# uber-research/deep-neuroevolution

Hardware: NVIDIA H100
Metric: env-steps/sec across ES population (whole box) (higher is better)
Workload: dtype f32

## Files before the change

### deep-neuroevolution_b200/csrc/conv_s2d.cu

```cuda
#include "common.cuh"
#include "forward.cuh"
#include "epilogue.cuh"
#include "wgmma.cuh"

using namespace wg;

namespace {

constexpr int S2D_MMA_THREADS = 256;
constexpr int S2D_CONV_WARPS = 4;
constexpr int S2D_CONV_THREADS = S2D_CONV_WARPS * 32;
constexpr int S2D_THREADS = 512;
constexpr int S2D_REGS_MMA = 176, S2D_REGS_AUX = 80;
constexpr int S2D_FRAME_BYTES = 84 * 84 * 4;
constexpr int S2D_FRAME_STRIDE = (S2D_FRAME_BYTES + 127) / 128 * 128;
constexpr int S2D_MAX_GROUPS = 8;
constexpr int S2D_MAX_BST = 8;
constexpr int S2D_SMEM_BUDGET = 222 * 1024;

constexpr int cmin(int a, int b) { return a < b ? a : b; }
constexpr int cmax(int a, int b) { return a > b ? a : b; }

struct S2dGeom {
    int S, PADB, W, KT, CIN, CP, NG, NPIX, PIXP, PARTS, LBO, GROUP_BYTES, IMG_BYTES, HIN;
};
__host__ __device__ constexpr S2dGeom s2d_geom(int CIN, int KS, int S, int HIN, int HOUT, int PAD, bool in_u8) {
    S2dGeom g{};
    const int HP = (HOUT - 1) * S + KS;
    g.S = S; g.PADB = PAD; g.W = HP / S; g.KT = KS / S; g.CIN = CIN; g.CP = S * S * CIN; g.NG = g.CP / 16;
    g.NPIX = g.W * g.W; g.PIXP = (g.NPIX + 7) / 8 * 8; g.PARTS = in_u8 ? 1 : 2; g.LBO = g.PIXP * 16;
    g.GROUP_BYTES = g.PARTS * 2 * g.LBO; g.IMG_BYTES = g.NG * g.GROUP_BYTES; g.HIN = HIN;
    return g;
}

constexpr int s2d_taps_per_chunk(int ntap, int piece_stride) {
    int best = 1;
    for (int t = 1; t <= ntap; ++t)
        if (ntap % t == 0 && 2 * t * piece_stride <= 26000) best = t;
    return best;
}

template <int CIN, int COUT, int KS, int S, int HIN, int HOUT, int PAD, bool IN_U8>
struct S2dCfg {
    static constexpr S2dGeom G = s2d_geom(CIN, KS, S, HIN, HOUT, PAD, IN_U8);
    static_assert(((HOUT - 1) * S + KS) % S == 0 && KS % S == 0, "space-to-depth needs S | KS and S | padded size");
    static_assert(CIN % 4 == 0 && COUT % 16 == 0 && G.CP % 16 == 0 && G.NG <= S2D_MAX_GROUPS, "tile constraints");
    static constexpr int W = G.W, KT = G.KT, NTAP = KT * KT, NG = G.NG, PIXP = G.PIXP, LBO_A = G.LBO;
    static constexpr int PARTS = G.PARTS, GROUP_BYTES = G.GROUP_BYTES, IMG_BYTES = G.IMG_BYTES;
    static constexpr int MMAX = (HOUT - 1) * (W + 1);
    static constexpr int MT = MMAX / 64 + 1;
    static constexpr int NTW = (MT + 1) / 2;
    static constexpr int ACC = COUT / 2;
    static_assert(2 * NTW * ACC <= 128, "accumulators exceed the MMA warpgroups' register budget");
    static constexpr int MAXOFF = (KT - 1) * (W + 1);
    static constexpr int REACH = MT * 64 + MAXOFF;
    static constexpr int SLACK = REACH > PIXP ? ((REACH - PIXP) * 16 + 127) / 128 * 128 : 0;
    static constexpr int A_REGION = IMG_BYTES + SLACK;
    static constexpr int LBO_B = 2 * COUT * 16;
    static constexpr int PIECE = 16 * COUT * 4;
    static constexpr int PIECE_STRIDE = PIECE + 16;
    static constexpr int TPC = s2d_taps_per_chunk(NTAP, PIECE_STRIDE);
    static constexpr int NCPG = NTAP / TPC;
    static constexpr int NCH = NG * NCPG;
    static constexpr int B_TILE = TPC * 2 * LBO_B;
    static constexpr int RAW_BYTES = 2 * TPC * PIECE_STRIDE;
    static constexpr int BST_BYTES = (cmax(B_TILE, RAW_BYTES) + 127) / 128 * 128;
    static constexpr int FRAME_REGION = IN_U8 ? 2 * S2D_FRAME_STRIDE : 0;
    static constexpr int NSTB = cmin(S2D_MAX_BST, (S2D_SMEM_BUDGET - A_REGION - FRAME_REGION - 256) / BST_BYTES);
    static_assert(NSTB >= 2, "shared memory: B ring too shallow");
    static constexpr int SMEM_BYTES = A_REGION + NSTB * BST_BYTES + FRAME_REGION + 256;
    static constexpr int B_UNITS = COUT * TPC * 2;
    static constexpr int NGRP = 2;
    static constexpr int WPG = S2D_CONV_WARPS / NGRP, TG = 32 * WPG;
    static constexpr int B_UPT = (B_UNITS + TG - 1) / TG;
    static_assert(TG % COUT == 0 && NCH % NGRP == 0, "B unit map: a thread keeps its column; groups alternate chunks");
    static_assert(!IN_U8 || NCPG == 1, "the uint8 frame is staged per channel group by the group's (only) chunk");
};

struct S2dOut {
    float* base;
    int64_t slot_stride;
    int next_img;
    int nS, nPADB, nW, nPIXP, nHP;
    float* xc;
    int xc_ko;
};

__device__ __forceinline__ void store_split_pair(uint4* p_hi, uint4* p_lo, int word, float v0, float v1) {
    uint32_t hi, lo;
    split_f16x2(v0, v1, hi, lo);
    reinterpret_cast<uint32_t*>(p_hi)[word] = hi;
    reinterpret_cast<uint32_t*>(p_lo)[word] = lo;
}

template <int COUT, int HOUT, int W, int MT, int NTW, int ACC, bool IN_U8, int MODE, bool FAST>
__device__ __forceinline__ void s2d_epilogue(const float (&acc)[NTW][ACC], const float (&cor)[NTW][ACC], int w, int wq, int lane,
                                             const float* sb, const float* sm, const float* si, const float* sg, const float* se,
                                             int act, bool bn, const S2dOut& so, float* outp, int slot) {
    constexpr float IN_SCALE = IN_U8 ? (1.0f / 255.0f) : 1.0f;
    const bool next_img = MODE < 0 ? so.next_img != 0 : MODE > 0;
    const int nS = MODE > 0 ? MODE : so.nS;
#pragma unroll
    for (int j = 0; j < NTW; ++j) {
        const int t = w + 2 * j;
        if (t >= MT) continue;
#pragma unroll
        for (int h = 0; h < 2; ++h) {
            const int m = t * 64 + wq * 16 + (lane >> 2) + 8 * h;
            const int oy = m / W, ox = m - oy * W;
            if (oy >= HOUT || ox >= HOUT) continue;
#pragma unroll
            for (int i = 0; i < COUT / 8; ++i) {
                const int n = 8 * i + 2 * (lane & 3);
                float v[2];
#pragma unroll
                for (int e = 0; e < 2; ++e) {
                    float r = fmaf(cor[j][4 * i + 2 * h + e], F16_LO_INV, acc[j][4 * i + 2 * h + e]);
                    if (IN_U8) r *= IN_SCALE;
                    r += sb[n + e];
                    if (FAST) {
                        v[e] = fmaxf(r, 0.0f);
                    } else {
                        if (bn) r = (r - sm[n + e]) * si[n + e] * sg[n + e] + se[n + e];
                        v[e] = act == DNE_ACT_RELU ? fmaxf(r, 0.0f) : (act == DNE_ACT_TANH ? tanhf(r) : r);
                    }
                }
                if (!next_img) {
                    *reinterpret_cast<float2*>(outp + (int64_t)(oy * HOUT + ox) * COUT + n) = make_float2(v[0], v[1]);
                    if (so.xc) {
                        const int ko = ((oy * HOUT + ox) * COUT + 8 * i) >> 3;
                        uint4* xp = reinterpret_cast<uint4*>(so.xc) + ((int64_t)(slot >> 7) * so.xc_ko + ko) * 256 + (slot & 127);
                        store_split_pair(xp, xp + 128, lane & 3, v[0], v[1]);
                    }
                } else {
                    const int Y = oy + so.nPADB, X = ox + so.nPADB;
                    const int pix = (Y / nS) * so.nW + (X / nS);
                    const int pp = (Y % nS) * nS + (X % nS);
                    const int co = pp * (COUT / 8) + i;
                    uint4* p = reinterpret_cast<uint4*>(outp) + (size_t)((co >> 1) * 4 + (co & 1)) * so.nPIXP + pix;
                    store_split_pair(p, p + (size_t)2 * so.nPIXP, lane & 3, v[0], v[1]);
                }
            }
        }
    }
}

template <int CIN, int COUT, int KS, int S, int HIN, int HOUT, int PAD, bool IN_U8>
__global__ void __launch_bounds__(S2D_THREADS, 1)
conv_s2d_kernel(SlotArgs sa, int64_t off_w, LayerEpi epi, const void* __restrict__ in_base, int64_t in_slot_stride,
                S2dOut so, int n_slots, int vdiv, int in_mod) {
    using Cfg = S2dCfg<CIN, COUT, KS, S, HIN, HOUT, PAD, IN_U8>;
    constexpr int NG = Cfg::NG, NSTB = Cfg::NSTB, MT = Cfg::MT, NTW = Cfg::NTW, W = Cfg::W, KT = Cfg::KT;
    constexpr int TPC = Cfg::TPC, NCPG = Cfg::NCPG, NCH = Cfg::NCH;
    extern __shared__ uint8_t smem_raw[];
    uint8_t* smem = (uint8_t*)(((uintptr_t)smem_raw + 127) & ~(uintptr_t)127);
    __shared__ uint64_t a_full[NG], a_empty[NG], raw_full[NSTB], b_full[NSTB], b_empty[NSTB];
    __shared__ uint64_t frame_full[2], frame_empty[2];
    __shared__ __align__(16) float s_bias[2][COUT], s_mean[2][COUT], s_inv[2][COUT], s_gamma[2][COUT], s_beta[2][COUT];

    const int tid = threadIdx.x, warp = tid >> 5, lane = tid & 31;
    pdl_trigger();
    const uint32_t sA = smem_u32(smem), sB = sA + Cfg::A_REGION;
    uint8_t* const gB = smem + Cfg::A_REGION;
    uint8_t* const gFrame = gB + NSTB * Cfg::BST_BYTES;

    if (tid == 0) {
        for (int i = 0; i < NG; ++i) {
            mbar_init(&a_full[i], IN_U8 ? Cfg::WPG : 1);
            mbar_init(&a_empty[i], S2D_MMA_THREADS);
        }
        for (int i = 0; i < NSTB; ++i) {
            mbar_init(&raw_full[i], 1);
            mbar_init(&b_full[i], Cfg::WPG);
            mbar_init(&b_empty[i], S2D_MMA_THREADS);
        }
        for (int i = 0; i < 2; ++i) {
            mbar_init(&frame_full[i], 1);
            mbar_init(&frame_empty[i], S2D_CONV_WARPS);
        }
        fence_mbar_init();
    }
    __syncthreads();
    if (warp < 8) regs_inc<S2D_REGS_MMA>();
    else regs_dec<S2D_REGS_AUX>();

    if (warp < 8) {
        const int w = warp >> 2, wq = warp & 3;
        const int et = tid;
        const int act = epi.act;
        const bool bn = epi.bn != DNE_BN_NONE;
        float acc[NTW][Cfg::ACC], cor[NTW][Cfg::ACC];
        uint32_t cb = 0, it = 0;
        pdl_wait();
        for (int slot = blockIdx.x; slot < n_slots; slot += gridDim.x) {
            const int ms = slot / vdiv;
            if (!slot_active(sa, ms)) continue;
            const uint32_t pb = it & 1;
            {
                const float* th = slot_theta(sa, ms);
                const int64_t idx = sa.noise_idx[ms];
                const float s = sa.scale[ms];
                for (int c = et; c < COUT; c += S2D_MMA_THREADS) {
                    const ChanEpi ce = make_chan_epi(sa, epi, ms, COUT, c, th, idx, s);
                    s_bias[pb][c] = ce.bias; s_mean[pb][c] = ce.mean; s_inv[pb][c] = ce.inv; s_gamma[pb][c] = ce.gamma; s_beta[pb][c] = ce.beta;
                }
            }
            float* outp = so.base + slot * so.slot_stride;
            if (so.next_img) {
                const int nHP = so.nHP, no = COUT / 8;
                for (int b = et; b < nHP * nHP; b += S2D_MMA_THREADS) {
                    const int Y = b / nHP, X = b - Y * nHP;
                    if (Y >= so.nPADB && Y < so.nPADB + HOUT && X >= so.nPADB && X < so.nPADB + HOUT) continue;
                    const int pix = (Y / so.nS) * so.nW + (X / so.nS), pp = (Y % so.nS) * so.nS + (X % so.nS);
                    for (int q = 0; q < no; ++q) {
                        const int co = pp * no + q;
                        uint4* p = reinterpret_cast<uint4*>(outp) + (size_t)((co >> 1) * 4 + (co & 1)) * so.nPIXP + pix;
                        p[0] = make_uint4(0u, 0u, 0u, 0u);
                        p[(size_t)2 * so.nPIXP] = make_uint4(0u, 0u, 0u, 0u);
                    }
                }
            }
            for (int c = 0; c < NCH; ++c, ++cb) {
                const int g = c / NCPG, tc = c - g * NCPG;
                const uint32_t st = cb % NSTB;
                if (tc == 0) mbar_wait(&a_full[g], it & 1);
                mbar_wait(&b_full[st], (cb / NSTB) & 1);
                wgmma_fence();
#pragma unroll
                for (int tl = 0; tl < TPC; ++tl) {
                    const int tap = tc * TPC + tl;
                    const int toff = (tap / KT) * W + (tap % KT);
                    const uint64_t dB = smem_desc(sB + st * Cfg::BST_BYTES + tl * 2 * Cfg::LBO_B, Cfg::LBO_B, 128);
#pragma unroll
                    for (int j = 0; j < NTW; ++j) {
                        const int t = min(w + 2 * j, MT - 1);
                        const uint64_t dA = smem_desc(sA + g * Cfg::GROUP_BYTES + (t * 64 + toff) * 16, Cfg::LBO_A, 128);
                        const uint32_t first = (c | tl) != 0;
                        wgmma_f16<COUT>(acc[j], dA, dB, first);
                        wgmma_f16<COUT>(cor[j], dA, dB + (uint64_t)((COUT * 16) >> 4), first);
                        if (!IN_U8) wgmma_f16<COUT>(cor[j], dA + (uint64_t)((2 * Cfg::LBO_A) >> 4), dB, 1);
                    }
                }
                wgmma_commit();
                wgmma_wait<1>();
                if (c > 0) {
                    const int pg = (c - 1) / NCPG;
                    mbar_arrive(&b_empty[(cb - 1) % NSTB]);
                    if ((c - 1) - pg * NCPG == NCPG - 1) mbar_arrive(&a_empty[pg]);
                }
            }
            wgmma_wait<0>();
#pragma unroll
            for (int j = 0; j < NTW; ++j) {
                fence_regs<Cfg::ACC>(acc[j]);
                fence_regs<Cfg::ACC>(cor[j]);
            }
            mbar_arrive(&b_empty[(cb - 1) % NSTB]);
            mbar_arrive(&a_empty[NG - 1]);
            named_bar_sync(2, S2D_MMA_THREADS);
            {
                const float *sb = s_bias[pb], *sm = s_mean[pb], *si = s_inv[pb], *sg = s_gamma[pb], *se = s_beta[pb];
                const bool relu_only = !bn && act == DNE_ACT_RELU;
#define S2D_EPI(MODE, FAST)                                                                                              \
    s2d_epilogue<COUT, HOUT, W, MT, NTW, Cfg::ACC, IN_U8, MODE, FAST>(acc, cor, w, wq, lane, sb, sm, si, sg, se, act, bn, so, \
                                                                       outp, slot)
                constexpr int FAST_MODE = CIN == 32 ? 1 : 0;
                if (!IN_U8 && relu_only && (FAST_MODE == 0 ? !so.next_img : (so.next_img && so.nS == FAST_MODE)))
                    S2D_EPI(FAST_MODE, true);
                else S2D_EPI(-1, false);
#undef S2D_EPI
            }
            ++it;
        }
    } else if (warp == 12) {
        if (lane == 0) {
            pdl_wait();
            uint32_t it = 0;
            for (int slot = blockIdx.x; slot < n_slots; slot += gridDim.x) {
                if (!slot_active(sa, slot / vdiv)) continue;
                if (IN_U8) {
                    const uint32_t fb = it & 1;
                    mbar_wait(&frame_empty[fb], ((it >> 1) & 1) ^ 1);
                    mbar_arrive_expect_tx(&frame_full[fb], S2D_FRAME_BYTES);
                    const int fslot = in_mod > 0 ? slot % in_mod : slot;
                    bulk_g2s(gFrame + fb * S2D_FRAME_STRIDE, (const uint8_t*)in_base + fslot * in_slot_stride, S2D_FRAME_BYTES,
                             &frame_full[fb]);
                } else {
                    const uint8_t* src = (const uint8_t*)((const float*)in_base + slot * in_slot_stride);
                    for (int g = 0; g < NG; ++g) {
                        mbar_wait(&a_empty[g], (it & 1) ^ 1);
                        mbar_arrive_expect_tx(&a_full[g], Cfg::GROUP_BYTES);
                        bulk_g2s(smem + g * Cfg::GROUP_BYTES, src + (size_t)g * Cfg::GROUP_BYTES, Cfg::GROUP_BYTES, &a_full[g]);
                    }
                }
                ++it;
            }
        }
    } else if (warp == 13) {
        if (lane == 0) {
            uint32_t cb = 0;
            for (int slot = blockIdx.x; slot < n_slots; slot += gridDim.x) {
                const int ms = slot / vdiv;
                if (!slot_active(sa, ms)) continue;
                const float* th = slot_theta(sa, ms) + off_w;
                const float* nz = sa.noise + sa.noise_idx[ms] + off_w;
                const int a_t = (int)(((uintptr_t)th >> 2) & 3), a_n = (int)(((uintptr_t)nz >> 2) & 3);
                for (int c = 0; c < NCH; ++c, ++cb) {
                    const int g = c / NCPG, tc = c - g * NCPG;
                    const uint32_t st = cb % NSTB;
                    mbar_wait(&b_empty[st], ((cb / NSTB) & 1) ^ 1);
                    mbar_arrive_expect_tx(&raw_full[st], Cfg::RAW_BYTES);
                    uint8_t* dst = gB + st * Cfg::BST_BYTES;
                    const int cp = 16 * g, pp = cp / CIN, ci = cp % CIN, py = pp / S, px = pp % S;
#pragma unroll
                    for (int tl = 0; tl < TPC; ++tl) {
                        const int tap = tc * TPC + tl;
                        const int ty = tap / KT, tx = tap % KT;
                        const int kk = ((ty * S + py) * KS + (tx * S + px)) * CIN + ci;
                        bulk_g2s(dst + tl * Cfg::PIECE_STRIDE, th + (int64_t)kk * COUT - a_t, Cfg::PIECE_STRIDE, &raw_full[st]);
                        bulk_g2s(dst + (TPC + tl) * Cfg::PIECE_STRIDE, nz + (int64_t)kk * COUT - a_n, Cfg::PIECE_STRIDE, &raw_full[st]);
                    }
                }
            }
        }
    } else if (warp < 12) {
        constexpr int TG = Cfg::TG, NGRP = Cfg::NGRP;
        const int ct = tid - S2D_MMA_THREADS;
        const int grp = ct / TG, tg = ct - grp * TG;
        {
            constexpr int Z0 = IN_U8 ? 0 : Cfg::IMG_BYTES, Z1 = Cfg::A_REGION;
            for (int i = Z0 / 16 + ct; i < Z1 / 16; i += S2D_CONV_THREADS) sts128(sA + i * 16, make_float4(0.f, 0.f, 0.f, 0.f));
            fence_proxy_async_smem();
            named_bar_sync(1, S2D_CONV_THREADS);
        }
        const int n = tg % COUT;
        constexpr int KQ_STEP = TG / COUT;
        const int kq0 = tg / COUT;
        uint32_t it = 0;
        for (int slot = blockIdx.x; slot < n_slots; slot += gridDim.x) {
            const int ms = slot / vdiv;
            if (!slot_active(sa, ms)) continue;
            const float* th = slot_theta(sa, ms) + off_w;
            const float* nz = sa.noise + sa.noise_idx[ms] + off_w;
            const int a_t = (int)(((uintptr_t)th >> 2) & 3), a_n = (int)(((uintptr_t)nz >> 2) & 3);
            const float s = sa.scale[ms];
            if (IN_U8) mbar_wait(&frame_full[it & 1], (it >> 1) & 1);
            for (int c = grp; c < NCH; c += NGRP) {
                const int g = c / NCPG;
                const uint32_t cb = it * NCH + c, st = cb % NSTB;
                if (IN_U8) {
                    static_assert(!IN_U8 || (CIN == 4 && S == 4 && HIN == 84), "uint8 staging is written for the 84x84x4 frame stack, stride 4");
                    const uint32_t frame = smem_u32(gFrame + (it & 1) * S2D_FRAME_STRIDE);
                    const int py = g;
                    mbar_wait(&a_empty[g], (it & 1) ^ 1);
                    for (int u = tg; u < 2 * W * W; u += TG) {
                        const int h = u / (W * W), pix = u - h * (W * W);
                        const int yq = pix / W, xq = pix - yq * W;
                        const int y = 4 * yq + py - PAD, x0 = 4 * xq + 2 * h - PAD;
                        if (y >= 0 && y < HIN && x0 >= 0 && x0 < HIN) {
                            uint32_t p0, p1;
                            asm volatile("ld.shared.v2.u32 {%0, %1}, [%2];" : "=r"(p0), "=r"(p1) : "r"(frame + (y * HIN + x0) * 4));
                            auto h2 = [](uint32_t lo8, uint32_t hi8) {
                                return (uint32_t)__half_as_ushort(__ushort2half_rn((unsigned short)lo8)) |
                                       ((uint32_t)__half_as_ushort(__ushort2half_rn((unsigned short)hi8)) << 16);
                            };
                            const uint4 row = make_uint4(h2(p0 & 255u, (p0 >> 8) & 255u), h2((p0 >> 16) & 255u, p0 >> 24),
                                                         h2(p1 & 255u, (p1 >> 8) & 255u), h2((p1 >> 16) & 255u, p1 >> 24));
                            sts128u(sA + g * Cfg::GROUP_BYTES + h * Cfg::LBO_A + pix * 16, row);
                        }
                    }
                    fence_proxy_async_smem();
                    __syncwarp();
                    if (lane == 0) {
                        mbar_arrive(&a_full[g]);
                        if (c + NGRP >= NCH) mbar_arrive(&frame_empty[it & 1]);
                    }
                }
                mbar_wait(&raw_full[st], (cb / NSTB) & 1);
                const uint32_t sBs = sB + st * Cfg::BST_BYTES;
                float w[Cfg::B_UPT][8];
#pragma unroll
                for (int i = 0; i < Cfg::B_UPT; ++i) {
                    const int kp = kq0 + i * KQ_STEP;
                    if (kp < TPC * 2) {
                        const uint32_t pt = sBs + (kp >> 1) * Cfg::PIECE_STRIDE + (uint32_t)((a_t + (8 * (kp & 1)) * COUT + n) * 4);
                        const uint32_t pn = sBs + (TPC + (kp >> 1)) * Cfg::PIECE_STRIDE + (uint32_t)((a_n + (8 * (kp & 1)) * COUT + n) * 4);
#pragma unroll
                        for (int j = 0; j < 8; ++j) w[i][j] = perturbed(lds32(pt + j * COUT * 4), s, lds32(pn + j * COUT * 4));
                    }
                }
                named_bar_sync(3 + grp, TG);
#pragma unroll
                for (int i = 0; i < Cfg::B_UPT; ++i) {
                    const int kp = kq0 + i * KQ_STEP;
                    if (kp < TPC * 2) {
                        uint4 hi, lo;
                        split_f16x8(w[i], hi, lo);
                        sts128u(sBs + kp * Cfg::LBO_B + n * 16, hi);
                        sts128u(sBs + kp * Cfg::LBO_B + (COUT + n) * 16, lo);
                    }
                }
                fence_proxy_async_smem();
                __syncwarp();
                if (lane == 0) mbar_arrive(&b_full[st]);
            }
            ++it;
        }
    }
}

template <int CIN, int COUT, int KS, int S, int HIN, int HOUT, int PAD, bool IN_U8>
int launch_s2d(const SlotArgs& sa, const dne_layer_desc& L, const LayerEpi& epi, const void* in, int64_t in_slot_stride,
               const S2dOut& so, int n_slots, int sm_count, cudaStream_t st, int vdiv, int in_mod) {
    using Cfg = S2dCfg<CIN, COUT, KS, S, HIN, HOUT, PAD, IN_U8>;
    auto kern = conv_s2d_kernel<CIN, COUT, KS, S, HIN, HOUT, PAD, IN_U8>;
    int dev = 0;
    cudaGetDevice(&dev);
    static bool attr_done[64] = {};
    if (dev < 64 && !attr_done[dev]) {
        if (cudaFuncSetAttribute(kern, cudaFuncAttributeMaxDynamicSharedMemorySize, Cfg::SMEM_BYTES) != cudaSuccess)
            return DNE_ERR_CUDA;
        attr_done[dev] = true;
    }
    const int grid = n_slots < sm_count ? n_slots : sm_count;
    if (dne_launch_chain(kern, dim3(grid), dim3(S2D_THREADS), (size_t)Cfg::SMEM_BYTES, st, !IN_U8 || g_dne_chain_ticks, sa, (int64_t)L.off_w, epi, in,
                         in_slot_stride, so, n_slots, vdiv, in_mod) != cudaSuccess)
        return DNE_ERR_CUDA;
    DNE_LAUNCHED(1);
    return 0;
}

bool shape_is(const dne_layer_desc& L, int cin, int cout, int ks, int stride, int hin, int hout, int pad) {
    return L.kind == DNE_CONV && L.cin == cin && L.cout == cout && L.ksize == ks && L.stride == stride && L.hin == hin &&
           L.hout == hout && L.pad == pad;
}

}

bool dne_s2d_supported(const dne_layer_desc& L, bool in_u8) {
    if (in_u8) return shape_is(L, 4, 32, 8, 4, 84, 21, 2) || shape_is(L, 4, 16, 8, 4, 84, 21, 2);
    return shape_is(L, 32, 64, 4, 2, 21, 11, 1) || shape_is(L, 16, 32, 4, 2, 21, 11, 1) || shape_is(L, 64, 64, 3, 1, 11, 11, 1);
}

size_t dne_s2d_image_bytes(const dne_layer_desc& L) {
    if (!dne_s2d_supported(L, false)) return 0;
    const S2dGeom g = s2d_geom(L.cin, L.ksize, L.stride, L.hin, L.hout, L.pad, false);
    return (size_t)g.IMG_BYTES;
}

void dne_s2d_image_geom(const dne_layer_desc& L, int* nS, int* nPADB, int* nW, int* nPIXP, int* nHP) {
    const S2dGeom g = s2d_geom(L.cin, L.ksize, L.stride, L.hin, L.hout, L.pad, false);
    *nS = g.S; *nPADB = g.PADB; *nW = g.W; *nPIXP = g.PIXP; *nHP = g.W * g.S;
}

int dne_launch_conv_layer_s2d(const SlotArgs& sa, const dne_layer_desc& L, const LayerEpi& epi, bool in_u8, const void* in,
                              int64_t in_slot_stride, float* out, int64_t out_slot_stride, const dne_layer_desc* next,
                              int n_slots, int sm_count, cudaStream_t st, float* xc, int vdiv, int in_mod) {
    S2dOut so;
    so.xc = next ? nullptr : xc;
    so.xc_ko = (L.hout * L.hout * L.cout) / 8;
    so.base = out;
    so.slot_stride = out_slot_stride;
    so.next_img = next ? 1 : 0;
    so.nS = so.nPADB = so.nW = so.nPIXP = so.nHP = 1;
    if (next) {
        const S2dGeom g = s2d_geom(next->cin, next->ksize, next->stride, next->hin, next->hout, next->pad, false);
        so.nS = g.S; so.nPADB = g.PADB; so.nW = g.W; so.nPIXP = g.PIXP; so.nHP = g.W * g.S;
    }
#define ARGS sa, L, epi, in, in_slot_stride, so, n_slots, sm_count, st, (vdiv < 1 ? 1 : vdiv), in_mod
    if (in_u8 && shape_is(L, 4, 32, 8, 4, 84, 21, 2)) return launch_s2d<4, 32, 8, 4, 84, 21, 2, true>(ARGS);
    if (in_u8 && shape_is(L, 4, 16, 8, 4, 84, 21, 2)) return launch_s2d<4, 16, 8, 4, 84, 21, 2, true>(ARGS);
    if (!in_u8 && shape_is(L, 32, 64, 4, 2, 21, 11, 1)) return launch_s2d<32, 64, 4, 2, 21, 11, 1, false>(ARGS);
    if (!in_u8 && shape_is(L, 16, 32, 4, 2, 21, 11, 1)) return launch_s2d<16, 32, 4, 2, 21, 11, 1, false>(ARGS);
    if (!in_u8 && shape_is(L, 64, 64, 3, 1, 11, 11, 1)) return launch_s2d<64, 64, 3, 1, 11, 11, 1, false>(ARGS);
#undef ARGS
    return DNE_ERR_UNSUP;
}
```

Before: 383,400.

## Stage conv epilogue through swizzled shared memory for vectorized output stores

The conv epilogue now writes the combined hi/lo accumulators into a per-warpgroup swizzled shared-memory staging tile, then reads them back row-wise so each thread handles a whole output pixel. That lets it emit float4 stores and 16-byte split-f16 packed stores, replacing the scattered 8-byte and 4-byte ones. The goal is to cut the cost of uncoalesced global writes. In exchange it reserves extra shared memory, which shrinks the B ring depth, and adds named barriers per tile. It also drops the specialized FAST/MODE template paths, so runtime branches on act/bn/next_img return.

```diff
diff --git a/deep-neuroevolution_b200/csrc/conv_s2d.cu b/deep-neuroevolution_b200/csrc/conv_s2d.cu
--- a/deep-neuroevolution_b200/csrc/conv_s2d.cu
+++ b/deep-neuroevolution_b200/csrc/conv_s2d.cu
@@ -66,9 +66,12 @@
     static constexpr int RAW_BYTES = 2 * TPC * PIECE_STRIDE;
     static constexpr int BST_BYTES = (cmax(B_TILE, RAW_BYTES) + 127) / 128 * 128;
     static constexpr int FRAME_REGION = IN_U8 ? 2 * S2D_FRAME_STRIDE : 0;
-    static constexpr int NSTB = cmin(S2D_MAX_BST, (S2D_SMEM_BUDGET - A_REGION - FRAME_REGION - 256) / BST_BYTES);
-    static_assert(NSTB >= 2, "shared memory: B ring too shallow");
-    static constexpr int SMEM_BYTES = A_REGION + NSTB * BST_BYTES + FRAME_REGION + 256;
+    static constexpr int STAGE_BYTES = 64 * COUT * 4;
+    static constexpr int STAGE_REGION = 2 * STAGE_BYTES;
+    static constexpr int NSTB = cmin(S2D_MAX_BST, (S2D_SMEM_BUDGET - A_REGION - FRAME_REGION - STAGE_REGION - 256) / BST_BYTES);
+    static_assert(NSTB >= 5, "shared memory: B ring too shallow to hide a stage's TMA -> conversion -> MMA cycle");
+    static constexpr int SMEM_BYTES = A_REGION + NSTB * BST_BYTES + FRAME_REGION + STAGE_REGION + 256;
+    static_assert(SMEM_BYTES <= S2D_SMEM_BUDGET, "shared memory budget");
     static constexpr int B_UNITS = COUT * TPC * 2;
     static constexpr int NGRP = 2;
     static constexpr int WPG = S2D_CONV_WARPS / NGRP, TG = 32 * WPG;
@@ -86,61 +89,89 @@
     int xc_ko;
 };
 
-__device__ __forceinline__ void store_split_pair(uint4* p_hi, uint4* p_lo, int word, float v0, float v1) {
-    uint32_t hi, lo;
-    split_f16x2(v0, v1, hi, lo);
-    reinterpret_cast<uint32_t*>(p_hi)[word] = hi;
-    reinterpret_cast<uint32_t*>(p_lo)[word] = lo;
-}
-
-template <int COUT, int HOUT, int W, int MT, int NTW, int ACC, bool IN_U8, int MODE, bool FAST>
-__device__ __forceinline__ void s2d_epilogue(const float (&acc)[NTW][ACC], const float (&cor)[NTW][ACC], int w, int wq, int lane,
-                                             const float* sb, const float* sm, const float* si, const float* sg, const float* se,
-                                             int act, bool bn, const S2dOut& so, float* outp, int slot) {
+template <int COUT>
+__device__ __forceinline__ int s2d_stage_swz(int r) {
+    static_assert(COUT == 16 || COUT % 32 == 0, "staging swizzle");
+    return COUT == 16 ? (r >> 1) & 1 : r & 3;
+}
+
+template <int COUT, int NTW, int ACC>
+__device__ __forceinline__ void s2d_stage_tile(const float (&acc)[NTW][ACC], const float (&cor)[NTW][ACC], int j, int wq,
+                                               int lane, uint32_t stage) {
+#pragma unroll
+    for (int jj = 0; jj < NTW; ++jj) {
+        if (jj != j) continue;
+#pragma unroll
+        for (int h = 0; h < 2; ++h) {
+            const int r = wq * 16 + (lane >> 2) + 8 * h;
+            const uint32_t row = stage + (uint32_t)(r * COUT + 2 * (lane & 3)) * 4;
+#pragma unroll
+            for (int i = 0; i < COUT / 8; ++i) {
+                const int k = 4 * i + 2 * h;
+                const float v0 = fmaf(cor[jj][k], F16_LO_INV, acc[jj][k]);
+                const float v1 = fmaf(cor[jj][k + 1], F16_LO_INV, acc[jj][k + 1]);
+                asm volatile("st.shared.v2.f32 [%0], {%1, %2};" ::"r"(row + (uint32_t)((i ^ s2d_stage_swz<COUT>(r)) * 32)),
+                             "f"(v0), "f"(v1) : "memory");
+            }
+        }
+    }
+}
+
+template <int COUT, int HOUT, int W, bool IN_U8>
+__device__ __forceinline__ void s2d_store_tile(int t, int k, uint32_t stage, const float* sb, const float* sm, const float* si,
+                                               const float* sg, const float* se, int act, bool bn, const S2dOut& so,
+                                               float* outp, int slot) {
     constexpr float IN_SCALE = IN_U8 ? (1.0f / 255.0f) : 1.0f;
-    const bool next_img = MODE < 0 ? so.next_img != 0 : MODE > 0;
-    const int nS = MODE > 0 ? MODE : so.nS;
-#pragma unroll
-    for (int j = 0; j < NTW; ++j) {
-        const int t = w + 2 * j;
-        if (t >= MT) continue;
-#pragma unroll
-        for (int h = 0; h < 2; ++h) {
-            const int m = t * 64 + wq * 16 + (lane >> 2) + 8 * h;
-            const int oy = m / W, ox = m - oy * W;
-            if (oy >= HOUT || ox >= HOUT) continue;
-#pragma unroll
-            for (int i = 0; i < COUT / 8; ++i) {
-                const int n = 8 * i + 2 * (lane & 3);
-                float v[2];
-#pragma unroll
-                for (int e = 0; e < 2; ++e) {
-                    float r = fmaf(cor[j][4 * i + 2 * h + e], F16_LO_INV, acc[j][4 * i + 2 * h + e]);
-                    if (IN_U8) r *= IN_SCALE;
-                    r += sb[n + e];
-                    if (FAST) {
-                        v[e] = fmaxf(r, 0.0f);
-                    } else {
-                        if (bn) r = (r - sm[n + e]) * si[n + e] * sg[n + e] + se[n + e];
-                        v[e] = act == DNE_ACT_RELU ? fmaxf(r, 0.0f) : (act == DNE_ACT_TANH ? tanhf(r) : r);
-                    }
-                }
-                if (!next_img) {
-                    *reinterpret_cast<float2*>(outp + (int64_t)(oy * HOUT + ox) * COUT + n) = make_float2(v[0], v[1]);
-                    if (so.xc) {
-                        const int ko = ((oy * HOUT + ox) * COUT + 8 * i) >> 3;
-                        uint4* xp = reinterpret_cast<uint4*>(so.xc) + ((int64_t)(slot >> 7) * so.xc_ko + ko) * 256 + (slot & 127);
-                        store_split_pair(xp, xp + 128, lane & 3, v[0], v[1]);
-                    }
-                } else {
-                    const int Y = oy + so.nPADB, X = ox + so.nPADB;
-                    const int pix = (Y / nS) * so.nW + (X / nS);
-                    const int pp = (Y % nS) * nS + (X % nS);
-                    const int co = pp * (COUT / 8) + i;
-                    uint4* p = reinterpret_cast<uint4*>(outp) + (size_t)((co >> 1) * 4 + (co & 1)) * so.nPIXP + pix;
-                    store_split_pair(p, p + (size_t)2 * so.nPIXP, lane & 3, v[0], v[1]);
-                }
-            }
+    constexpr int NO = COUT / 8;
+    const int ri = k & 63, m = t * 64 + ri;
+    const int oy = m / W, ox = m - oy * W;
+    if (oy >= HOUT || ox >= HOUT) return;
+    const uint32_t row = stage + (uint32_t)(ri * COUT) * 4;
+    const int swz = s2d_stage_swz<COUT>(ri);
+    uint4* p_hi = nullptr;
+    int lo_off = 0, step = 0;
+    if (so.next_img) {
+        const int Y = oy + so.nPADB, X = ox + so.nPADB;
+        const int pix = (Y / so.nS) * so.nW + (X / so.nS);
+        const int pp = (Y % so.nS) * so.nS + (X % so.nS);
+        p_hi = reinterpret_cast<uint4*>(outp) + (int64_t)pp * (NO / 2) * 4 * so.nPIXP + pix;
+        lo_off = 2 * so.nPIXP;
+        step = so.nPIXP;
+    } else if (so.xc) {
+        p_hi = reinterpret_cast<uint4*>(so.xc) + ((int64_t)(slot >> 7) * so.xc_ko + (oy * HOUT + ox) * NO) * 256 + (slot & 127);
+        lo_off = 128;
+        step = 256;
+    }
+#pragma unroll 1
+    for (int o = k >> 6; o < NO; o += 2) {
+        float v[8];
+        {
+            float4 x0, x1;
+            const uint32_t a = row + (uint32_t)((o ^ swz) * 32);
+            asm volatile("ld.shared.v4.f32 {%0, %1, %2, %3}, [%4];" : "=f"(x0.x), "=f"(x0.y), "=f"(x0.z), "=f"(x0.w) : "r"(a));
+            asm volatile("ld.shared.v4.f32 {%0, %1, %2, %3}, [%4];" : "=f"(x1.x), "=f"(x1.y), "=f"(x1.z), "=f"(x1.w) : "r"(a + 16));
+            v[0] = x0.x; v[1] = x0.y; v[2] = x0.z; v[3] = x0.w; v[4] = x1.x; v[5] = x1.y; v[6] = x1.z; v[7] = x1.w;
+        }
+#pragma unroll
+        for (int e = 0; e < 8; ++e) {
+            const int n = 8 * o + e;
+            float r = v[e];
+            if (IN_U8) r *= IN_SCALE;
+            r += sb[n];
+            if (bn) r = (r - sm[n]) * si[n] * sg[n] + se[n];
+            v[e] = act == DNE_ACT_RELU ? fmaxf(r, 0.0f) : (act == DNE_ACT_TANH ? tanhf(r) : r);
+        }
+        if (!so.next_img) {
+            float4* dst = reinterpret_cast<float4*>(outp + (int64_t)(oy * HOUT + ox) * COUT + 8 * o);
+            dst[0] = make_float4(v[0], v[1], v[2], v[3]);
+            dst[1] = make_float4(v[4], v[5], v[6], v[7]);
+        }
+        if (p_hi) {
+            const int po = so.next_img ? ((o >> 1) * 4 + (o & 1)) * step : o * step;
+            uint4 hi, lo;
+            split_f16x8(v, hi, lo);
+            p_hi[po] = hi;
+            p_hi[po + lo_off] = lo;
         }
     }
 }
@@ -163,6 +194,7 @@
     const uint32_t sA = smem_u32(smem), sB = sA + Cfg::A_REGION;
     uint8_t* const gB = smem + Cfg::A_REGION;
     uint8_t* const gFrame = gB + NSTB * Cfg::BST_BYTES;
+    uint8_t* const gStage = gFrame + Cfg::FRAME_REGION;
 
     if (tid == 0) {
         for (int i = 0; i < NG; ++i) {
@@ -260,15 +292,16 @@
             named_bar_sync(2, S2D_MMA_THREADS);
             {
                 const float *sb = s_bias[pb], *sm = s_mean[pb], *si = s_inv[pb], *sg = s_gamma[pb], *se = s_beta[pb];
-                const bool relu_only = !bn && act == DNE_ACT_RELU;
-#define S2D_EPI(MODE, FAST)                                                                                              \
-    s2d_epilogue<COUT, HOUT, W, MT, NTW, Cfg::ACC, IN_U8, MODE, FAST>(acc, cor, w, wq, lane, sb, sm, si, sg, se, act, bn, so, \
-                                                                       outp, slot)
-                constexpr int FAST_MODE = CIN == 32 ? 1 : 0;
-                if (!IN_U8 && relu_only && (FAST_MODE == 0 ? !so.next_img : (so.next_img && so.nS == FAST_MODE)))
-                    S2D_EPI(FAST_MODE, true);
-                else S2D_EPI(-1, false);
-#undef S2D_EPI
+                const uint32_t stage = smem_u32(gStage) + w * Cfg::STAGE_BYTES;
+#pragma unroll 1
+                for (int j = 0; j < NTW; ++j) {
+                    const int t = w + 2 * j;
+                    if (t >= MT) break;
+                    if (j > 0) named_bar_sync(5 + w, 128);
+                    s2d_stage_tile<COUT, NTW, Cfg::ACC>(acc, cor, j, wq, lane, stage);
+                    named_bar_sync(5 + w, 128);
+                    s2d_store_tile<COUT, HOUT, W, IN_U8>(t, tid & 127, stage, sb, sm, si, sg, se, act, bn, so, outp, slot);
+                }
             }
             ++it;
         }
```

Measured after the change: 403,900 (median of 6 runs). 5.3% higher.
